# xuyuan/waymo_2d_tracking

Measured on AMD Instinct MI355X. Metric: end-to-end frames/sec (detect+SORT) on 1920x1280 Waymo frames, higher is better.
Workload: dtype f32; 1 GPU; Cascade R-CNN X152-32x8d-FPN dconv (random-init, fp32, batch 1) on synthetic 1920x1280x3 frames -> top-100 detections/frame -> SORT (max_age 2, min_hits 0, all boxes tracked; trackers resident for the whole segment); 5 cameras x 2 frames per step per GPU; 1x1 and dense 3x3 convolutions: f32 operands as exact 3 x bf16 splits, six cross terms on the bf16 matrix cores, f32 accumulate (csrc/det_gemm_s; stage=e2e, parallelism=sequence-shard x1

## Files before the change

### include/waymodet.h

```cpp
#ifndef WAYMODET_H
#define WAYMODET_H
#include <stddef.h>
#include <stdint.h>
#ifdef __cplusplus
extern "C" {
#endif

int wd_roi_pool_fpn_f32(const float* const* feats, const int32_t* heights, const int32_t* widths,
                        const float* scales, int n_levels, int channels, int batch,
                        const float* rois, int n_rois, int pooled, int min_level, int canonical_level,
                        float canonical_size, float* out, void* stream);

size_t wd_nms_workspace(int n);
int wd_select_kept(const uint8_t* keep_mask, const uint8_t* valid, const int64_t* order, int n, int cap, int64_t* out_idx,
                   int32_t* count, void* stream);
int wd_nms_sorted_f32(const float* boxes, const int32_t* idxs, int n, float iou_threshold,
                      uint8_t* keep_mask, int32_t* n_keep, void* workspace, size_t workspace_bytes, void* stream);

size_t wd_gemm_nt_workspace(int M, int N, int K);
int wd_gemm_nt_ws_f32(const float* A, const float* Bt, const float* bias, const float* residual, int relu, int M, int N, int K,
                      float* C, void* workspace, size_t workspace_bytes, void* stream);

int wd_gemm_lt_f32(const float* a, const float* w, const float* bias, const float* residual, float* out, int m, int n, int k,
                   int relu, void* workspace, size_t workspace_bytes, void* stream);
int wd_gemm_lt_plan_info(int m, int n, int k, int relu, int has_bias, int has_residual, float* best_us, int* candidates);
size_t wd_gemm_split_packed_bytes(int N, int K);
int wd_gemm_split_pack_weight(const float* w, int N, int K, void* packed, void* stream);
int wd_gemm_split_pack_weight_strided(const float* w, int N, int K, long stride_n, long stride_k, void* packed, void* stream);
typedef struct WdSplitPackDesc {
    const float* src;
    void* dst;
    long s_n, s_c, s_kh, s_kw;
    long first_block;
    int N, K, C, ksize, flip, reserved;
} WdSplitPackDesc;
int wd_gemm_split_pack_batch(const WdSplitPackDesc* descs_device, int count, long total_blocks, void* stream);
size_t wd_gemm_split_workspace(long M, int N, int K);
int wd_gemm_split_f32(const float* a, long lda, const void* packed_w, const float* bias, const float* residual, float* out, long ldc,
                      int M, int N, int K, int relu, void* workspace, size_t workspace_bytes, void* stream);
int wd_conv_split_f32(const float* x, int batch, int H, int W, int C, const void* packed_w, int ksize, int stride, int pad, const float* bias,
                      const float* residual, float* out, int N, int relu, void* workspace, size_t workspace_bytes, void* stream);
int wd_gemm_split_supported(const float* a, long lda, const float* bias, const float* residual, const float* out, long ldc, long M, int N, int K);
int wd_conv_split_position_major(int batch, int H, int W, int ksize, int stride, int pad);
typedef struct WdSplitIO {
    const float* a;
    long lda;
    const void* a_planes;
    const float* residual;
    const void* residual_planes;
    float* out;
    void* out_planes;
    long ldc;
} WdSplitIO;
size_t wd_split_planes_bytes(long M, int K);
int wd_split_planes_pack_f32(const float* a, long lda, long M, int K, void* planes, void* stream);
int wd_split_planes_unpack_f32(const void* planes, long M, int K, float* out, long ldo, void* stream);
int wd_gemm_split_io(const WdSplitIO* io, const void* packed_w, const float* bias, int M, int N, int K, int relu, void* workspace,
                     size_t workspace_bytes, void* stream);
int wd_nms_segmented_f32(const float* boxes, const int32_t* idxs, const int32_t* seg_offsets, int n_seg, float iou_threshold,
                         uint8_t* keep_mask, int32_t* n_keep, void* workspace, size_t workspace_bytes, void* stream);

size_t wd_rpn_topk_workspace(const int* n_per_level, int n_levels, int k);
int wd_rpn_topk_decode_f32(const float* const* logits, const float* const* deltas, const float* const* anchors,
                           const int* n_per_level, int n_levels, int k, float img_h, float img_w, float scale_clamp,
                           float* out_boxes, float* out_scores, int32_t* out_group, uint8_t* out_valid, void* workspace,
                           size_t workspace_bytes, void* stream);
int wd_sort_candidates_f32(const float* boxes, const float* scores, const int32_t* group, const uint8_t* valid,
                           const uint8_t* valid2 , int n, float* out_boxes, float* out_scores, int32_t* out_group, uint8_t* out_valid, int64_t* out_order,
                           void* stream);
int wd_box_candidates_f32(const float* boxes, const float* s0, const float* s1, const float* s2, const int32_t* n_valid, int rows,
                          int num_classes, float score_thresh, float img_h, float img_w, float* out_boxes, float* out_scores,
                          int32_t* out_group, uint8_t* out_valid, int64_t* out_order, void* stream);
int wd_gather_kept_f32(const uint8_t* keep, const uint8_t* valid, const float* boxes, const float* scores, const int64_t* order,
                       int n, int cap, int num_classes, float* out_boxes, float* out_scores, int64_t* out_class, int32_t* count,
                       void* stream);
int wd_detections_to_wire(const float* boxes, const float* scores, const int64_t* classes, const int32_t* count, int n, int in_w,
                          int in_h, int hflip, int out_w, int out_h, double* xywhs, int32_t* category, void* stream);

size_t wd_deform_packed_weight_floats(int c_in, int c_out, int groups);
int wd_deform_pack_weight(const float* weight_oihw, int c_in, int c_out, int groups, float* packed, void* stream);
const char* wd_deform_conv3x3_variant(int c_in, int groups, int stride, int pad, int has_offset);
int wd_deform_conv3x3_f32(const float* x, const float* offset, const float* mask, const float* packed_weight,
                          const float* scale, const float* bias, int relu,
                          int batch, int h, int w, int c_in, int c_out, int groups, int stride, int pad,
                          float* y, void* stream);
int wd_deform_conv3x3_hint_f32(const float* x, const float* offset, const float* mask, const float* packed_weight,
                               const float* scale, const float* bias, int relu, int batch, int h, int w, int c_in,
                               int c_out, int groups, int stride, int pad, int far_offsets, float* y, void* stream);
size_t wd_deform_table_bytes(int batch, int h, int w);
int wd_deform_offsets_table_f32(const float* partial, int ld, const float* bias, int batch, int h, int w, float* offsets,
                                void* table, void* stream);
int wd_deform_conv3x3_tab_f32(const float* x, const float* offset, const float* mask, const float* packed_weight,
                              const float* scale, const float* bias, int relu, int batch, int h, int w, int c_in,
                              int c_out, int groups, int stride, int pad, int far_offsets, const void* table, float* y,
                              void* stream);
// ... 57 lines not shown
```

### waymo_2d_tracking_amd/csrc/det_gemm_split.hip

```cpp
#include "common.h"
#include "../../include/waymodet.h"
#include <cstdlib>
#include <cstring>

namespace {

using bf16x8 = __attribute__((ext_vector_type(8))) __bf16;
using bf16x2 = __attribute__((ext_vector_type(2))) __bf16;
using f32x2 = __attribute__((ext_vector_type(2))) float;
using f32x16 = __attribute__((ext_vector_type(16))) float;
using u32x4 = __attribute__((ext_vector_type(4))) unsigned;

constexpr int BK = 64;
constexpr int BN = 256;
constexpr int NTHREADS = 512;
constexpr int CHUNK = 6144;

struct SplitArgs {
    const float* a;
    const unsigned char* ap;
    const uint4* w;
    const float* bias;
    const float* residual;
    const unsigned char* resp;
    float* out;
    unsigned char* outp;
    long lda, ldc;
    int M, N, K, relu;
    int tiles_m, tiles_n;
    int splitk;
    float* part;
    long long* stamps;
    int H, W, C, Ho, Wo, stride, pad, ksize;
};

__device__ __forceinline__ unsigned pk_bf16(float a, float b) {
    const f32x2 v = {a, b};
    return __builtin_bit_cast(unsigned, __builtin_convertvector(v, bf16x2));
}

__device__ __forceinline__ void split_pair(float x0, float x1, unsigned& h, unsigned& m, unsigned& l) {
    h = pk_bf16(x0, x1);
    const float r0 = x0 - __uint_as_float(h << 16), r1 = x1 - __uint_as_float(h & 0xffff0000u);
    m = pk_bf16(r0, r1);
    const float s0 = r0 - __uint_as_float(m << 16), s1 = r1 - __uint_as_float(m & 0xffff0000u);
    l = pk_bf16(s0, s1);
}

__device__ __forceinline__ float bf_lo(unsigned v) { return __uint_as_float(v << 16); }
__device__ __forceinline__ float bf_hi(unsigned v) { return __uint_as_float(v & 0xffff0000u); }

__device__ __forceinline__ size_t planes_offset(int row, int col, int ncols) {
    return ((size_t)(row >> 5) * (size_t)(ncols >> 5) + (size_t)(col >> 5)) * CHUNK +
           (size_t)((row & 31) * 64 + ((((col >> 3) & 3) ^ ((row >> 2) & 3)) << 4) + ((col >> 2) & 1) * 8);
}

// ... 490 lines not shown
    if ((j_) < ND) { dma_piece(kt + 3, (unsigned)wr, (j_)); }
    RD(rofs0, 2) RD(rofs0, 1) RD(rofs0, 0)
    SB;
    int cur = 0, nxt = BUF, nx2 = 2 * BUF, wr = 3 * BUF;
    for (int kt = 0; kt < nk; ++kt) {
        const int a1 = cur + rofs1, a0n = nxt + rofs0;
        WAITW(0, ND + 3);
        MF(2, 0, 0) RD(a1, 2) SB;
        MF(1, 1, 0) SB;
        MF(1, 0, 0) RD(a1, 1) SB;
        MF(0, 2, 0) SB;
        MF(0, 1, 0) SB;
        MF(0, 0, 0) RD(a1, 0) w_load(2 * kt + 2, 0); SB;
        WAITW(1, 3);
        MF(2, 0, 1) RD(a0n, 2) SB;
        MF(1, 1, 1) DMA(0) DMA(3) SB;
        MF(1, 0, 1) RD(a0n, 1) SB;
        MF(0, 2, 1) DMA(1) DMA(4) SB;
        MF(0, 1, 1) DMA(2) SB;
        MF(0, 0, 1) RD(a0n, 0) w_load(2 * kt + 3, 1); SB;
        __builtin_amdgcn_s_barrier();
        SB;
        const int t = cur; cur = nxt; nxt = nx2; nx2 = wr; wr = t;
    }
#undef DMA
#undef WAITW
#ifdef WD_DEBUG
    if (p.stamps) t_epi = __builtin_amdgcn_s_memtime();
#endif
    asm volatile("s_waitcnt vmcnt(0) lgkmcnt(0)" ::: "memory");
    __builtin_amdgcn_s_barrier();
    if (p.splitk > 1) {
        SplitArgs q = p;
        q.out = p.part + (size_t)kz * p.M * p.N;
        q.ldc = p.N;
        q.bias = nullptr; q.residual = nullptr; q.resp = nullptr; q.outp = nullptr; q.relu = 0;
        split_epilogue<MT>(q, smem, acc, m0, n0, wave, lane, p.M);
    } else {
        split_epilogue<MT>(p, smem, acc, m0, n0, wave, lane, p.M);
    }
#ifdef WD_DEBUG
    if (p.stamps && tid == 0) {
        long long* o = p.stamps + 8 * (long)blockIdx.x;
        o[0] = t_start; o[1] = t_main; o[2] = t_epi; o[3] = __builtin_amdgcn_s_memtime();
        o[4] = id_stamp; o[5] = __builtin_amdgcn_s_getreg(20  | (0 << 6) | (3 << 11));
        o[6] = r_start; o[7] = __builtin_amdgcn_s_memrealtime();
    }
#endif
}
#undef SB
#undef MF
#undef RD

__global__ __launch_bounds__(256) void split_planes_pack_kernel(const float* __restrict__ a, long lda, int M, int K, unsigned char* __restrict__ out, long total) {
    const long t = (long)blockIdx.x * 256 + threadIdx.x;
    if (t >= total) return;
    const int k8 = K / 8;
    const int row = (int)(t / k8), kq = (int)(t - (long)row * k8);
    float4 v0 = make_float4(0.f, 0.f, 0.f, 0.f), v1 = v0;
    if (row < M) {
        const float4* s = reinterpret_cast<const float4*>(a + (size_t)row * lda + 8 * kq);
        v0 = s[0]; v1 = s[1];
    }
    unsigned h[4], m[4], l[4];
    split_pair(v0.x, v0.y, h[0], m[0], l[0]); split_pair(v0.z, v0.w, h[1], m[1], l[1]);
    split_pair(v1.x, v1.y, h[2], m[2], l[2]); split_pair(v1.z, v1.w, h[3], m[3], l[3]);
    unsigned char* q = out + planes_offset(row, 8 * kq, K);
    *reinterpret_cast<uint4*>(q) = make_uint4(h[0], h[1], h[2], h[3]);
    *reinterpret_cast<uint4*>(q + 2048) = make_uint4(m[0], m[1], m[2], m[3]);
    *reinterpret_cast<uint4*>(q + 4096) = make_uint4(l[0], l[1], l[2], l[3]);
}

__global__ __launch_bounds__(256) void split_planes_unpack_kernel(const unsigned char* __restrict__ planes, int M, int K, float* __restrict__ out, long ldo, long total) {
    const long t = (long)blockIdx.x * 256 + threadIdx.x;
    if (t >= total) return;
    const int k8 = K / 8;
    const int row = (int)(t / k8), kq = (int)(t - (long)row * k8);
    const unsigned char* q = planes + planes_offset(row, 8 * kq, K);
    const uint4 h = *reinterpret_cast<const uint4*>(q), m = *reinterpret_cast<const uint4*>(q + 2048), l = *reinterpret_cast<const uint4*>(q + 4096);
    float4* d = reinterpret_cast<float4*>(out + (size_t)row * ldo + 8 * kq);
    d[0] = make_float4((bf_lo(h.x) + bf_lo(m.x)) + bf_lo(l.x), (bf_hi(h.x) + bf_hi(m.x)) + bf_hi(l.x), (bf_lo(h.y) + bf_lo(m.y)) + bf_lo(l.y),
                       (bf_hi(h.y) + bf_hi(m.y)) + bf_hi(l.y));
    d[1] = make_float4((bf_lo(h.z) + bf_lo(m.z)) + bf_lo(l.z), (bf_hi(h.z) + bf_hi(m.z)) + bf_hi(l.z), (bf_lo(h.w) + bf_lo(m.w)) + bf_lo(l.w),
                       (bf_hi(h.w) + bf_hi(m.w)) + bf_hi(l.w));
}

__global__ __launch_bounds__(256) void gemm_split_pack_kernel(const float* __restrict__ w, int N, int K, long sn, long sk, uint4* __restrict__ out, long total) {
    const long t = (long)blockIdx.x * 256 + threadIdx.x;
    if (t >= total) return;
    const int k8 = K / 8;
    const int n = (int)(t / k8), kq = (int)(t - (long)n * k8);
    float v[8];
#pragma unroll
    for (int e = 0; e < 8; ++e) v[e] = n < N ? w[(size_t)n * sn + (size_t)(8 * kq + e) * sk] : 0.f;
    unsigned h[4], m[4], l[4];
#pragma unroll
    for (int e = 0; e < 4; ++e) split_pair(v[2 * e], v[2 * e + 1], h[e], m[e], l[e]);
    const int nt = n >> 5, ks = kq >> 1, ln = (n & 31) + 32 * (kq & 1);
    uint4* dst = out + ((size_t)nt * (K / 16) + ks) * 192 + ln;
    dst[0] = make_uint4(h[0], h[1], h[2], h[3]);
    dst[64] = make_uint4(m[0], m[1], m[2], m[3]);
    dst[128] = make_uint4(l[0], l[1], l[2], l[3]);
}

__global__ __launch_bounds__(256) void gemm_split_pack_batch_kernel(const WdSplitPackDesc* __restrict__ descs, int count) {
    int lo = 0, hi = count - 1;
// ... 155 lines not shown
    if (pl.splitk > 1 && workspace_bytes < (size_t)pl.splitk * a.M * a.N * sizeof(float)) pl = pick_plan(a.M, a.N, a.K, false);
    const int mt = pl.mt;
    a.splitk = pl.splitk;
    a.part = pl.splitk > 1 ? (float*)workspace : nullptr;
    a.tiles_m = (a.M + 32 * mt - 1) / (32 * mt);
    a.tiles_n = (a.N + BN - 1) / BN;
    int rc;
    switch (mt) {
        case 2: rc = launch<2, MODE>(a, stream); break;
        case 3: rc = launch<3, MODE>(a, stream); break;
        case 4: rc = launch<4, MODE>(a, stream); break;
        case 6: rc = launch<6, MODE>(a, stream); break;
        default: rc = launch<5, MODE>(a, stream); break;
    }
    if (rc != WT_OK || a.splitk == 1) return rc;
    const long mn4 = (long)a.M * a.N / 4;
    hipLaunchKernelGGL(gemm_split_reduce_kernel, dim3((unsigned)((mn4 + 255) / 256)), dim3(256), 0, stream, (const float4*)a.part, a.splitk, mn4, a.N / 4,
                       (const float4*)a.bias, a.residual, a.resp, a.ldc, a.relu, a.out, a.outp);
    WT_HIP(hipGetLastError());
    return WT_OK;
}

int dispatch_position_major(SplitArgs& a, hipStream_t stream) {
#ifdef WD_DEBUG
    a.stamps = g_stamps;
#endif
    const int maps = a.M / (a.H * a.W), kc = a.C / 32;
    const long tn = (a.N + BN - 1) / BN;
    const long ni = (long)(a.H - 2) * (a.W - 2), ne = 2l * (a.W - 2) + 2l * (a.H - 2);
    int best = 4;
    double best_t = 1e30;
    static const int forced_mt = experiment_knob("WD_SPLIT_MT");
    for (int mt = MT_MAX; mt >= MT_MIN; --mt) {
        if (forced_mt >= MT_MIN && forced_mt <= MT_MAX && mt != forced_mt) continue;
        const long nch = (maps + 32 * mt - 1) / (32 * mt);
        const double eff = (mt == 4 || mt == 5) ? 1.0 : 1.24;
        auto tile = [&](int taps) { return mt * taps * kc * 0.52 * eff + 2.0 + mt; };
        const double work = (double)nch * tn * (ni * tile(9) + ne * tile(6) + 4 * tile(4)) / 256.0;
        const double t = work > tile(9) ? work : tile(9);
        if (t < best_t * 0.97) { best_t = t; best = mt; }
    }
    a.splitk = 1; a.part = nullptr;
    a.tiles_m = a.H * a.W * ((maps + 32 * best - 1) / (32 * best));
    a.tiles_n = (int)tn;
    switch (best) {
        case 4: return launch<4, 3>(a, stream);
        case 6: return launch<6, 3>(a, stream);
        default: return launch<5, 3>(a, stream);
    }
}

bool misaligned(const void* p) { return (reinterpret_cast<uintptr_t>(p) & 15) != 0; }

}

extern "C" {

#ifdef WD_DEBUG
int wd_gemm_split_debug_stamps(long long* buf) {
    g_stamps = buf;
    return WT_OK;
}
#endif

size_t wd_gemm_split_packed_bytes(int N, int K) {
    if (N <= 0 || K <= 0 || (K % BK)) return 0;
    return (size_t)((N + 31) / 32) * 32 * (size_t)K * 6;
}

int wd_gemm_split_pack_weight_strided(const float* w, int N, int K, long stride_n, long stride_k, void* packed, void* stream_) {
    WT_TRY(wt::ensure_device());
    if (!w || !packed || N <= 0 || K <= 0 || (K % BK)) {
        wt::set_error("wd_gemm_split_pack_weight: K must be a positive multiple of %d (N=%d K=%d)", BK, N, K);
        return WT_ERR_INVALID;
    }
    const long total = (long)((N + 31) / 32) * 32 * (K / 8);
    hipLaunchKernelGGL(gemm_split_pack_kernel, dim3((unsigned)((total + 255) / 256)), dim3(256), 0, (hipStream_t)stream_, w, N, K, stride_n, stride_k,
                       (uint4*)packed, total);
    WT_HIP(hipGetLastError());
    return WT_OK;
}

int wd_gemm_split_pack_weight(const float* w, int N, int K, void* packed, void* stream_) {
    return wd_gemm_split_pack_weight_strided(w, N, K, (long)K, 1, packed, stream_);
}

int wd_gemm_split_pack_batch(const WdSplitPackDesc* descs_device, int count, long total_blocks, void* stream_) {
    WT_TRY(wt::ensure_device());
    if (count <= 0 || total_blocks <= 0) return WT_OK;
    if (!descs_device || total_blocks >= (1l << 31)) {
        wt::set_error("wd_gemm_split_pack_batch: NULL descriptor array or too many workgroups (%ld)", total_blocks);
        return WT_ERR_INVALID;
    }
    hipLaunchKernelGGL(gemm_split_pack_batch_kernel, dim3((unsigned)total_blocks), dim3(256), 0, (hipStream_t)stream_, descs_device, count);
    WT_HIP(hipGetLastError());
    return WT_OK;
}

size_t wd_gemm_split_workspace(long M, int N, int K) {
    if (M <= 0 || N <= 0 || K <= 0 || (K % BK) || (N % 32)) return 0;
    const Plan pl = pick_plan(M, N, K, true);
    return pl.splitk > 1 ? (size_t)pl.splitk * M * N * sizeof(float) : 0;
}

int wd_gemm_split_supported(const float* a, long lda, const float* bias, const float* residual, const float* out, long ldc, long M, int N, int K) {
    return M > 0 && N > 0 && K > 0 && (K % BK) == 0 && (N % 32) == 0 && (lda & 3) == 0 && (ldc & 3) == 0 && lda >= K && ldc >= N && !misaligned(a) &&
           !misaligned(bias) && !misaligned(residual) && !misaligned(out) && M < (1l << 31) && M * lda < (1l << 31);
}

int wd_gemm_split_f32(const float* a, long lda, const void* packed_w, const float* bias, const float* residual, float* out, long ldc,
                      int M, int N, int K, int relu, void* workspace, size_t workspace_bytes, void* stream_) {
    WT_TRY(wt::ensure_device());
    if (M <= 0 || N <= 0) return WT_OK;
    if (!a || !packed_w || !out || misaligned(packed_w) || !wd_gemm_split_supported(a, lda, bias, residual, out, ldc, M, N, K)) {
        wt::set_error("wd_gemm_split_f32: needs K %% %d == 0, N %% 32 == 0, 16-byte aligned rows and M * lda < 2^31 (M=%d N=%d K=%d lda=%ld)", BK, M, N,
                      K, lda);
        return WT_ERR_INVALID;
    }
    SplitArgs s{};
    s.a = a; s.w = (const uint4*)packed_w; s.bias = bias; s.residual = residual; s.out = out;
    s.lda = lda; s.ldc = ldc; s.M = M; s.N = N; s.K = K; s.relu = relu;
    return dispatch<0>(s, workspace, workspace_bytes, (hipStream_t)stream_);
}

size_t wd_split_planes_bytes(long M, int K) {
    if (M <= 0 || K <= 0 || (K % 32)) return 0;
    return (size_t)((M + 31) / 32) * (size_t)(K / 32) * CHUNK;
}

int wd_split_planes_pack_f32(const float* a, long lda, long M, int K, void* planes, void* stream_) {
    WT_TRY(wt::ensure_device());
    if (!a || !planes || M <= 0 || M >= (1l << 31) || K <= 0 || (K % 32) || (lda & 3) || lda < K || misaligned(a) || misaligned(planes)) {
        wt::set_error("wd_split_planes_pack_f32: needs K %% 32 == 0 and 16-byte aligned rows (M=%ld K=%d lda=%ld)", M, K, lda);
        return WT_ERR_INVALID;
    }
    const long total = ((M + 31) / 32) * 32 * (K / 8);
    hipLaunchKernelGGL(split_planes_pack_kernel, dim3((unsigned)((total + 255) / 256)), dim3(256), 0, (hipStream_t)stream_, a, lda, (int)M, K,
                       (unsigned char*)planes, total);
    WT_HIP(hipGetLastError());
    return WT_OK;
}

int wd_split_planes_unpack_f32(const void* planes, long M, int K, float* out, long ldo, void* stream_) {
    WT_TRY(wt::ensure_device());
    if (!out || !planes || M <= 0 || M >= (1l << 31) || K <= 0 || (K % 32) || (ldo & 3) || ldo < K || misaligned(out) || misaligned(planes)) {
        wt::set_error("wd_split_planes_unpack_f32: needs K %% 32 == 0 and 16-byte aligned rows (M=%ld K=%d ldo=%ld)", M, K, ldo);
        return WT_ERR_INVALID;
    }
    const long total = M * (K / 8);
    hipLaunchKernelGGL(split_planes_unpack_kernel, dim3((unsigned)((total + 255) / 256)), dim3(256), 0, (hipStream_t)stream_, (const unsigned char*)planes,
                       (int)M, K, out, ldo, total);
    WT_HIP(hipGetLastError());
    return WT_OK;
}

int wd_gemm_split_io(const WdSplitIO* io, const void* packed_w, const float* bias, int M, int N, int K, int relu, void* workspace,
                     size_t workspace_bytes, void* stream_) {
    WT_TRY(wt::ensure_device());
    if (M <= 0 || N <= 0) return WT_OK;
    if (!io || !packed_w || misaligned(packed_w) || (!io->a && !io->a_planes) || (io->a && io->a_planes) || (!io->out && !io->out_planes) ||
        (io->residual && io->residual_planes) || K <= 0 || (K % BK) || (N % 32) || misaligned(io->a_planes) || misaligned(io->residual_planes) ||
        misaligned(io->out_planes) ||
        !wd_gemm_split_supported(io->a ? io->a : (const float*)packed_w, io->a ? io->lda : K, bias, io->residual, io->out, io->ldc ? io->ldc : N, M, N, K)) {
        wt::set_error("wd_gemm_split_io: exactly one of a / a_planes, at least one of out / out_planes, at most one residual form; K %% %d == 0, "
                      "N %% 32 == 0, 16-byte aligned pointers and rows (M=%d N=%d K=%d)", BK, M, N, K);
        return WT_ERR_INVALID;
    }
    SplitArgs s{};
    s.a = io->a; s.ap = (const unsigned char*)io->a_planes; s.w = (const uint4*)packed_w; s.bias = bias;
    s.residual = io->residual; s.resp = (const unsigned char*)io->residual_planes; s.out = io->out; s.outp = (unsigned char*)io->out_planes;
    s.lda = io->a ? io->lda : K; s.ldc = io->ldc ? io->ldc : N; s.M = M; s.N = N; s.K = K; s.relu = relu;
    return io->a ? dispatch<0>(s, workspace, workspace_bytes, (hipStream_t)stream_) : dispatch<2>(s, workspace, workspace_bytes, (hipStream_t)stream_);
}

int wd_conv_split_position_major(int batch, int H, int W, int ksize, int stride, int pad) {
// ... 25 lines not shown
```

### waymo_2d_tracking_amd/detnet/nn/cascade_rcnn.py

```python
import math
import os

import torch
from torch import nn
import torch.nn.functional as F

from . import ops

BLOCKS = (3, 8, 36, 3)
STAGE_CH = (256, 512, 1024, 2048)
GROUPS = 32
PIXEL_MEAN = (103.530, 116.280, 123.675)
PIXEL_STD = (57.375, 57.120, 58.395)
SCALE_CLAMP = math.log(1000.0 / 16)


FUSED_TRAINING_EPILOGUES = True


SPLIT_GEMM = os.environ.get('WD_SPLIT_GEMM', '1') != '0'


OFFSET_SPLIT_MIN_ROWS = 30000


SPLIT_PLANES = os.environ.get('WD_SPLIT_PLANES', '0') == '1'
SPLIT_PLANES_MIN_CH = int(os.environ.get('WD_SPLIT_PLANES_MIN_CH', '1024'))


class PlanesAct:

    def __init__(self, planes, n, h, w, c):
        self.planes, self.n, self.h, self.w, self.c = planes, n, h, w, c


DECISION_LOG = None


def _split_ok(cin, cout):
    return SPLIT_GEMM and cin % 64 == 0 and cout % 32 == 0


class _PackedSplit:

    def __init__(self):
        self.buf = None
        self.key = None

    def get(self, weight):
        key = (weight.device, weight._version, weight.data_ptr())
        if self.buf is None or self.key != key:
            self.buf = ops.split_pack_weight(weight)
            self.key = key
        return self.buf


def _msra(shape, gen, fan_out=True):
    w = torch.empty(shape)
    fan = shape[0] * shape[2] * shape[3] if fan_out else shape[1] * shape[2] * shape[3]
    return w.normal_(0, math.sqrt(2.0 / fan), generator=gen)


class Conv1x1(nn.Module):

    def __init__(self, cin, cout, gen, bn_scale=1.0, bias=False):
        super().__init__()
        w = _msra((cout, cin, 1, 1), gen).view(cout, cin)
        s = bn_scale / math.sqrt(1.0 + 1e-5) if not bias else 1.0
        self.weight = nn.Parameter(w * s, requires_grad=False)
        self.bias = nn.Parameter(torch.zeros(cout), requires_grad=False)
        self._split = _PackedSplit()

    def forward(self, x, relu=False, residual=None, stride=1):
        if not torch.is_grad_enabled() and x.is_cuda and _split_ok(self.weight.shape[1], self.weight.shape[0]):
            pw = self._split.get(self.weight)
            cout = self.weight.shape[0]
# ... 55 lines not shown
            return ops.conv_split(x, self._split.get(self.weight), self.weight.shape[0], self.weight.shape[2], self.stride, self.pad,
                                  self.bias, None, relu)
        if not torch.is_grad_enabled() and self.weight.shape[0] % 4 == 0:
            y = F.conv2d(x, self.weight, None, self.stride, self.pad, 1, self.groups)
            if y.is_contiguous(memory_format=torch.channels_last):
                n, c, h, w = y.shape
                ops.bias_relu_(y.permute(0, 2, 3, 1).reshape(n * h * w, c), self.bias, relu)
                return y
            y = y + self.bias.view(1, -1, 1, 1)
            return F.relu_(y) if relu else y
        if (torch.is_grad_enabled() and ops.SPLIT_TRAIN and x.is_cuda and self.groups == 1 and self.weight.shape[2] in (1, 3)
                and _split_ok(self.weight.shape[1], self.weight.shape[0])):
            return ops.ConvSplitFn.apply(x, self.weight, self.bias, self.stride, self.pad, relu)
        y = F.conv2d(x, self.weight, self.bias, self.stride, self.pad, 1, self.groups)
        return F.relu_(y) if relu else y


class Bottleneck(nn.Module):

    def __init__(self, cin, cout, stride, deform, gen, offset_std):
        super().__init__()
        width = cout
        self.stride, self.deform = stride, deform
        self.shortcut = Conv1x1(cin, cout, gen) if cin != cout else None
        self.conv1 = Conv1x1(cin, width, gen)
        if deform:
            self.conv2_offset = ConvBN(width, 18, 3, stride, 1, 1, gen, bias=True)
            self.conv2_offset.weight.data.normal_(0, offset_std, generator=gen)
            w = _msra((width, width // GROUPS, 3, 3), gen)
            self.conv2_weight = nn.Parameter(w, requires_grad=False)
            self.conv2_scale = nn.Parameter(torch.full((width,), 1.0 / math.sqrt(1.0 + 1e-5)), requires_grad=False)
            self.conv2_bias = nn.Parameter(torch.zeros(width), requires_grad=False)
            self._packed = None
        else:
            self.conv2_weight = nn.Parameter(_msra((width, width // GROUPS, 3, 3), gen), requires_grad=False)
            self.conv2_scale = nn.Parameter(torch.full((width,), 1.0 / math.sqrt(1.0 + 1e-5)), requires_grad=False)
            self.conv2_bias = nn.Parameter(torch.zeros(width), requires_grad=False)
            self._packed = None
        self.conv3 = Conv1x1(width, cout, gen, bn_scale=0.25)

    def packed_weight(self):
        v = self.conv2_weight._version
        if self._packed is None or self._packed.device != self.conv2_weight.device or getattr(self, '_packed_v', -1) != v:
            self._packed = ops.deform_pack_weight(self.conv2_weight, GROUPS)
            self._packed_v = v
        return self._packed

    def offset_conv(self, x, deform_table=False, stride=1):
        w = self.conv2_offset.weight
        if getattr(self, '_off_w2', None) is None or self._off_w2.device != w.device or self._off_v != w._version:
            self._off_w2 = ops.tap_gemm_weight(w)
            self._off_v = w._version
        split = None
        if x.shape[0] * x.shape[2] * x.shape[3] >= OFFSET_SPLIT_MIN_ROWS and x.is_cuda and _split_ok(w.shape[1], 32):
            if getattr(self, '_off_split', None) is None or self._off_split_key != (w.device, w._version):
                w32 = ops.tap_gemm_weight(w, align=32)
                self._off_split, self._off_split_key = (ops.split_pack_weight(w32), w32.shape[0]), (w.device, w._version)
            split = self._off_split
        return ops.conv3x3_few(x, self._off_w2, self.conv2_offset.bias, 18, stride, deform_table, split=split)

    def forward(self, x, emit_planes=False):
        if isinstance(x, PlanesAct) or emit_planes:
            return self._forward_planes(x, emit_planes)
        sc = x if self.shortcut is None else self.shortcut(x, stride=self.stride)
        out = self.conv1(x, relu=True)
        rec = DECISION_LOG
        if rec is not None:
            out1, offset = out, None
        if self.deform and torch.is_grad_enabled():
            offset = self.conv2_offset(out)
            if FUSED_TRAINING_EPILOGUES and not (self.conv2_scale.requires_grad or self.conv2_bias.requires_grad):
                out = ops.DeformConvFn.apply(out, offset, self.conv2_weight, GROUPS, self.stride, 1, self.conv2_scale, self.conv2_bias, True)
            else:
                out = ops.DeformConvFn.apply(out, offset, self.conv2_weight, GROUPS, self.stride, 1)
                out = F.relu(out * self.conv2_scale.view(1, -1, 1, 1) + self.conv2_bias.view(1, -1, 1, 1))
        elif self.deform:
            table = None
            if self.stride == 1 and self.conv2_weight.shape[1] in (16, 32):
                offset, table = self.offset_conv(out, deform_table=True)
            else:
                offset = self.offset_conv(out, stride=self.stride)
            out = ops.deform_conv3x3(out, offset, self.packed_weight(), GROUPS, self.stride, 1, self.conv2_scale,
                                     self.conv2_bias, relu=True, table=table)
        else:
            out = ops.deform_conv3x3(out, None, self.packed_weight(), GROUPS, self.stride, 1, self.conv2_scale,
                                     self.conv2_bias, relu=True)
        if rec is None:
            return self.conv3(out, relu=True, residual=sc)
        out3 = self.conv3(out, relu=True, residual=sc)
        rec.append((out1.detach().clone(), None if offset is None else offset.detach().clone(), out.detach().clone(), out3.detach().clone(), self.stride))
        return out3


def _bottleneck_forward_planes(self, x, emit_planes):
    in_planes = isinstance(x, PlanesAct)
    cout = self.conv3.weight.shape[0]
    if in_planes:
        assert self.shortcut is None and self.stride == 1
        n, h, w, cin = x.n, x.h, x.w, x.c
        m = n * h * w
        o1, _ = ops.gemm_split_io(m, self.conv1.weight.shape[0], cin, self.conv1._split.get(self.conv1.weight), a_planes=x.planes, bias=self.conv1.bias, relu=True)
        out = o1.view(n, h, w, -1).permute(0, 3, 1, 2)
        sc = None
    else:
        sc = x if self.shortcut is None else self.shortcut(x, stride=self.stride)
        out = self.conv1(x, relu=True)
    table = None
    if self.stride == 1 and self.conv2_weight.shape[1] in (16, 32):
        offset, table = self.offset_conv(out, deform_table=True)
    else:
# ... 317 lines not shown
```

### waymo_2d_tracking_amd/detnet/nn/ops.py

```python
import ctypes as C
import os

import torch

from ... import _lib


EVENT_LOG = None


_RAW_STREAM = getattr(torch._C, '_cuda_getCurrentRawStream', None)
_RAW_DEVICE = getattr(torch._C, '_cuda_getDevice', None)


def _stream():
    if _RAW_STREAM is not None and _RAW_DEVICE is not None:
        return C.c_void_p(_RAW_STREAM(_RAW_DEVICE()))
    return C.c_void_p(torch.cuda.current_stream().cuda_stream)


def _p(t):
    return C.c_void_p(t.data_ptr()) if t is not None else None


# ... 177 lines not shown
    n, c, h, w = x.shape
    out = torch.empty((n, c, 2 * h, 2 * w), dtype=torch.float32, device=x.device, memory_format=torch.channels_last)
    _lib.check(_lib.lib().wd_upsample2x_nhwc_f32(_p(x), C.c_int(n), C.c_int(h), C.c_int(w), C.c_int(c), _p(out), _stream()),
               'wd_upsample2x_nhwc_f32')
    return out


def groupnorm_relu_(x, weight, bias, groups, eps=1e-5, relu=True):
    assert x.is_contiguous(memory_format=torch.channels_last) and x.dtype == torch.float32
    r, c, h, w = x.shape
    _lib.check(_lib.lib().wd_groupnorm_relu_nhwc_f32(_p(x), _p(weight), _p(bias), C.c_int(r), C.c_int(h * w), C.c_int(c),
                                                     C.c_int(groups), C.c_float(eps), C.c_int(1 if relu else 0), _stream()),
               'wd_groupnorm_relu_nhwc_f32')
    return x


class GroupNormReluFn(torch.autograd.Function):

    @staticmethod
    def forward(ctx, x, weight, bias, groups, eps, relu):
        x = _nhwc(x)
        r, c, h, w = x.shape
        y = torch.empty_like(x, memory_format=torch.channels_last)
        _lib.check(_lib.lib().wd_groupnorm_relu_out_nhwc_f32(_p(x), _p(y), _p(weight), _p(bias), C.c_int(r), C.c_int(h * w), C.c_int(c),
                                                             C.c_int(groups), C.c_float(eps), C.c_int(1 if relu else 0), _stream()),
                   'wd_groupnorm_relu_out_nhwc_f32')
        ctx.save_for_backward(x, weight, bias)
        ctx.cfg = (groups, eps, bool(relu))
        return y

    @staticmethod
    def backward(ctx, dy):
        x, weight, bias = ctx.saved_tensors
        groups, eps, relu = ctx.cfg
        dy = _nhwc(dy)
        r, c, h, w = x.shape
        dx = torch.empty_like(x, memory_format=torch.channels_last)
        dg = torch.empty(c, dtype=torch.float32, device=x.device)
        db = torch.empty(c, dtype=torch.float32, device=x.device)
        _lib.check(_lib.lib().wd_groupnorm_relu_bwd_nhwc_f32(_p(x), _p(dy), _p(weight), _p(bias), C.c_int(r), C.c_int(h * w), C.c_int(c),
                                                             C.c_int(groups), C.c_float(eps), C.c_int(1 if relu else 0), _p(dx), _p(dg), _p(db),
                                                             _stream()), 'wd_groupnorm_relu_bwd_nhwc_f32')
        return dx, dg, db, None, None, None


def tap_gemm_weight(weight, align=16):
    n_out, c = weight.shape[0], weight.shape[1]
    ld = (9 * n_out + align - 1) // align * align
    w2 = torch.zeros((ld, c), dtype=torch.float32, device=weight.device)
    w2[:9 * n_out] = weight.detach().float().permute(2, 3, 0, 1).reshape(9 * n_out, c)
    return w2


def conv3x3_few(x, w2, bias, n_out, stride=1, deform_table=False, split=None):
    x = _nhwc(x)
    n, c, h, w = x.shape
    a = x.permute(0, 2, 3, 1).reshape(n * h * w, c)
    if split is not None:
        packed, ld = split
        partial = gemm_split(a, packed, ld)
        ld_partial = ld
    else:
        partial = torch.mm(a, w2.t())
        ld_partial = w2.shape[0]
    ho, wo = (h - 1) // stride + 1, (w - 1) // stride + 1
    out = torch.empty((n, n_out, ho, wo), dtype=torch.float32, device=x.device, memory_format=torch.channels_last)
    if deform_table:
        assert n_out == 18 and stride == 1
        lib = _lib.lib()
        table = torch.empty(int(lib.wd_deform_table_bytes(C.c_int(n), C.c_int(h), C.c_int(w))), dtype=torch.uint8, device=x.device)
        _lib.check(lib.wd_deform_offsets_table_f32(_p(partial), C.c_int(ld_partial), _p(bias), C.c_int(n), C.c_int(h), C.c_int(w),
                                                   _p(out), _p(table), _stream()), 'wd_deform_offsets_table_f32')
        return out, table
    _lib.check(_lib.lib().wd_tap_shift_add_f32(_p(partial), C.c_int(ld_partial), C.c_int(n_out), _p(bias), C.c_int(n), C.c_int(h),
                                               C.c_int(w), C.c_int(stride), _p(out), _stream()), 'wd_tap_shift_add_f32')
    return out


_LT_WS = {}


def gemm_lt(a, weight, bias=None, residual=None, relu=False, out=None):
    m, k = a.shape
    n = weight.shape[0]
    assert a.is_contiguous() and weight.is_contiguous() and weight.shape[1] == k
    if out is None:
        out = torch.empty((m, n), dtype=torch.float32, device=a.device)
    assert out.is_contiguous() and (residual is None or residual.is_contiguous())
    key = (a.device, torch.cuda.current_stream().cuda_stream)
    ws = _LT_WS.get(key)
    if ws is None:
        ws = _LT_WS[key] = torch.empty(64 << 20, dtype=torch.uint8, device=a.device)
    _lib.check(_lib.lib().wd_gemm_lt_f32(_p(a), _p(weight), _p(bias), _p(residual), _p(out), C.c_int(m), C.c_int(n), C.c_int(k),
                                         C.c_int(1 if relu else 0), _p(ws), C.c_size_t(ws.numel()), _stream()), 'wd_gemm_lt_f32')
    return out


def _split_log_begin():
    if EVENT_LOG is None:
        return None
    e0 = torch.cuda.Event(enable_timing=True)
    e0.record()
    return e0


def _split_log_end(e0, tag, m, n, k):
    if e0 is None:
        return
    e1 = torch.cuda.Event(enable_timing=True)
    e1.record()
    EVENT_LOG.append((tag, 12.0 * m * n * k, e0, e1))


_SPLIT_WS_BYTES = {}
# ... 661 lines not shown
```

Measured before the change: 43.72 frames/s.

## Add thin split-bf16 GEMM for deform offset taps with stride-2 parity classes

Adds a dedicated thin GEMM kernel for the 18-channel deformable-offset 3x3 tap GEMM (N<=192). It splits A into bf16 planes in shared memory and uses 32x32x16 bf16 MFMA with double buffering. For stride-2 convs, input pixels are grouped into four parity classes, and each class computes only the taps that contribute to strided outputs, skipping unneeded tap products. The row-count threshold for using the split path is removed, so small levels also use it. This adds extra launches per stride-2 conv and scattered output writes.

Result: no change. 43.42 frames/s (-0.7%).

```diff
diff --git a/include/waymodet.h b/include/waymodet.h
--- a/include/waymodet.h
+++ b/include/waymodet.h
@@ -41,6 +41,9 @@
 int wd_conv_split_f32(const float* x, int batch, int H, int W, int C, const void* packed_w, int ksize, int stride, int pad, const float* bias,
                       const float* residual, float* out, int N, int relu, void* workspace, size_t workspace_bytes, void* stream);
 int wd_gemm_split_supported(const float* a, long lda, const float* bias, const float* residual, const float* out, long ldc, long M, int N, int K);
+int wd_gemm_split_thin_f32(const float* a, long lda, const void* packed_w, float* partial, int ld, int M, int N, int K, void* stream);
+int wd_offset_taps_s2_split_f32(const float* x, int batch, int H, int W, int C, const void* const* packed_w, int n_out, float* partial, int ld,
+                                void* stream);
 int wd_conv_split_position_major(int batch, int H, int W, int ksize, int stride, int pad);
 typedef struct WdSplitIO {
     const float* a;
diff --git a/waymo_2d_tracking_amd/csrc/det_gemm_split.hip b/waymo_2d_tracking_amd/csrc/det_gemm_split.hip
--- a/waymo_2d_tracking_amd/csrc/det_gemm_split.hip
+++ b/waymo_2d_tracking_amd/csrc/det_gemm_split.hip
@@ -2,6 +2,7 @@
 #include "../../include/waymodet.h"
 #include <cstdlib>
 #include <cstring>
+#include <type_traits>
 
 namespace {
 
@@ -598,6 +599,148 @@
 #undef MF
 #undef RD
 
+struct ThinArgs {
+    const float* a;
+    const uint4* w;
+    float* out;
+    long lda;
+    int M, K, ld;
+    int ncb, ncols;
+    int H, W, hc, wc, py, px;
+    int group, ntaps;
+    unsigned taps;
+};
+
+__device__ __forceinline__ long thin_row(const ThinArgs& p, int m) {
+    if (p.H == 0) return m;
+    const int hw = p.hc * p.wc;
+    const int b = m / hw, r = m - b * hw;
+    const int yy = r / p.wc, xx = r - yy * p.wc;
+    return ((long)b * p.H + 2 * yy + p.py) * p.W + 2 * xx + p.px;
+}
+
+#define WD_THIN_VGPR_FLOOR "v167"
+
+template <int RB>
+__global__ __launch_bounds__(NTHREADS) void gemm_split_thin_kernel(const ThinArgs p) {
+    constexpr int BM = 32 * RB;
+    constexpr int PLANE = BM * 64;
+    constexpr int BUF = 3 * PLANE;
+    constexpr int NLD = RB / 2;
+    constexpr int CG = 8 / RB;
+    __shared__ __attribute__((aligned(16))) unsigned char smem[2 * BUF];
+    asm volatile("" ::: WD_THIN_VGPR_FLOOR);
+    const int tid = threadIdx.x, lane = tid & 63;
+    const int wave = __builtin_amdgcn_readfirstlane(tid >> 6);
+    const int m0 = blockIdx.x * BM;
+    const int rb = wave % RB, cg = wave / RB;
+    const int per = p.ncb / CG, rem = p.ncb % CG;
+    const int nj = per + (cg < rem ? 1 : 0);
+    const int cb0 = cg * per + (cg < rem ? cg : rem);
+    const int nk = p.K / 32;
+
+    const int sq = tid & 7;
+    const float* arow[NLD];
+    int soff[NLD];
+#pragma unroll
+    for (int i = 0; i < NLD; ++i) {
+        const int r = (tid >> 3) + 64 * i;
+        int m = m0 + r;
+        m = m < p.M ? m : p.M - 1;
+        arow[i] = p.a + thin_row(p, m) * p.lda + 4 * sq;
+        soff[i] = r * 64 + ((((sq >> 1) ^ ((r >> 2) & 3))) << 4) + (sq & 1) * 8;
+    }
+    auto a_fetch = [&](int kt, int i) -> float4 {
+        kt = kt < nk ? kt : nk - 1;
+        return *reinterpret_cast<const float4*>(arow[i] + (size_t)kt * 32);
+    };
+    auto a_store = [&](int bufoff, int i, const float4& v) {
+        unsigned h0, m0_, l0, h1, m1, l1;
+        split_pair(v.x, v.y, h0, m0_, l0);
+        split_pair(v.z, v.w, h1, m1, l1);
+        unsigned char* b = smem + bufoff + soff[i];
+        *reinterpret_cast<uint2*>(b) = make_uint2(h0, h1);
+        *reinterpret_cast<uint2*>(b + PLANE) = make_uint2(m0_, m1);
+        *reinterpret_cast<uint2*>(b + 2 * PLANE) = make_uint2(l0, l1);
+    };
+    float4 anext[NLD];
+#pragma unroll
+    for (int i = 0; i < NLD; ++i) a_store(0, i, a_fetch(0, i));
+#pragma unroll
+    for (int i = 0; i < NLD; ++i) anext[i] = a_fetch(1, i);
+
+    const int rr = lane & 31, rg = lane >> 5;
+    const int ro0 = (rb * 32 + rr) * 64 + ((((0 + rg) ^ ((rr >> 2) & 3))) << 4);
+    const int ro1 = (rb * 32 + rr) * 64 + ((((2 + rg) ^ ((rr >> 2) & 3))) << 4);
+
+    auto run = [&](auto njc) {
+        constexpr int NJ = decltype(njc)::value;
+        constexpr int NA = NJ > 0 ? NJ : 1;
+        f32x16 acc[NA];
+#pragma unroll
+        for (int j = 0; j < NA; ++j)
+#pragma unroll
+            for (int e = 0; e < 16; ++e) acc[j][e] = 0.f;
+        const uint4* wq[NA];
+#pragma unroll
+        for (int j = 0; j < NA; ++j) wq[j] = p.w + (size_t)(cb0 + j) * (size_t)(p.K / 16) * 192 + lane;
+        bf16x8 wf[2][NA][3];
+        auto w_load = [&](int sub, int slot) {
+            sub = sub < 2 * nk ? sub : 2 * nk - 1;
+#pragma unroll
+            for (int j = 0; j < NJ; ++j)
+#pragma unroll
+                for (int pl = 0; pl < 3; ++pl) wf[slot][j][pl] = __builtin_bit_cast(bf16x8, wq[j][(size_t)sub * 192 + pl * 64]);
+        };
+        auto sub_step = [&](int aoff, int slot) {
+            bf16x8 af[3];
+#pragma unroll
+            for (int pl = 0; pl < 3; ++pl) af[pl] = *reinterpret_cast<const bf16x8*>(smem + aoff + pl * PLANE);
+#define TERM(pa, pb)                                                                                          \
+    _Pragma("unroll") for (int j = 0; j < NJ; ++j)                                                          \
+        acc[j] = __builtin_amdgcn_mfma_f32_32x32x16_bf16(af[pa], wf[slot][j][pb], acc[j], 0, 0, 0);
+            TERM(2, 0) TERM(1, 1) TERM(1, 0) TERM(0, 2) TERM(0, 1) TERM(0, 0)
+#undef TERM
+        };
+        w_load(0, 0);
+        __syncthreads();
+        for (int kt = 0; kt < nk; ++kt) {
+            const int cur = (kt & 1) * BUF, nxt = BUF - cur;
+            if (kt + 1 < nk) {
+#pragma unroll
+                for (int i = 0; i < NLD; ++i) a_store(nxt, i, anext[i]);
+            }
+#pragma unroll
+            for (int i = 0; i < NLD; ++i) anext[i] = a_fetch(kt + 2, i);
+            if (NJ > 0) {
+                w_load(2 * kt + 1, 1);
+                sub_step(cur + ro0, 0);
+                w_load(2 * kt + 2, 0);
+                sub_step(cur + ro1, 1);
+            }
+            __syncthreads();
+        }
+#pragma unroll
+        for (int j = 0; j < NJ; ++j) {
+            const int col = (cb0 + j) * 32 + rr;
+            if (col >= p.ncols) continue;
+            int oc = col;
+            if (p.ntaps > 0) {
+                const int ti = col / p.group;
+                oc = (int)((p.taps >> (4 * ti)) & 15u) * p.group + (col - ti * p.group);
+            }
+#pragma unroll
+            for (int e = 0; e < 16; ++e) {
+                const int m = m0 + rb * 32 + (e & 3) + 8 * (e >> 2) + 4 * rg;
+                if (m < p.M) p.out[(size_t)thin_row(p, m) * p.ld + oc] = acc[j][e];
+            }
+        }
+    };
+    if (nj == 2) run(std::integral_constant<int, 2>{});
+    else if (nj == 1) run(std::integral_constant<int, 1>{});
+    else run(std::integral_constant<int, 0>{});
+}
+
 __global__ __launch_bounds__(256) void split_planes_pack_kernel(const float* __restrict__ a, long lda, int M, int K, unsigned char* __restrict__ out, long total) {
     const long t = (long)blockIdx.x * 256 + threadIdx.x;
     if (t >= total) return;
@@ -859,6 +1002,30 @@
 
 bool misaligned(const void* p) { return (reinterpret_cast<uintptr_t>(p) & 15) != 0; }
 
+template <int RB>
+int launch_thin(const ThinArgs& a, hipStream_t stream) {
+    const void* fn = reinterpret_cast<const void*>(gemm_split_thin_kernel<RB>);
+    static wt::OncePerDevice attr;
+    const int dev = wt::device_index();
+    if (attr.needed(dev)) {
+        WT_TRY(occupancy_guard(fn, RB));
+        attr.mark(dev);
+    }
+    hipLaunchKernelGGL((gemm_split_thin_kernel<RB>), dim3((unsigned)((a.M + 32 * RB - 1) / (32 * RB))), dim3(NTHREADS), 0, stream, a);
+    WT_HIP(hipGetLastError());
+    return WT_OK;
+}
+
+int dispatch_thin(ThinArgs& a, hipStream_t stream) {
+    a.ncb = (a.ncols + 31) / 32;
+    return a.ncb >= 4 ? launch_thin<2>(a, stream) : launch_thin<4>(a, stream);
+}
+
+bool thin_args_bad(const float* a, long lda, const void* packed_w, const float* partial, int ld, long M, int N, int K) {
+    return !a || !packed_w || !partial || misaligned(a) || misaligned(packed_w) || M <= 0 || M >= (1l << 31) || N <= 0 || N > 192 || ld < N || K <= 0 ||
+           (K % BK) || (lda & 3) || lda < K;
+}
+
 }
 
 extern "C" {
@@ -928,6 +1095,48 @@
     s.a = a; s.w = (const uint4*)packed_w; s.bias = bias; s.residual = residual; s.out = out;
     s.lda = lda; s.ldc = ldc; s.M = M; s.N = N; s.K = K; s.relu = relu;
     return dispatch<0>(s, workspace, workspace_bytes, (hipStream_t)stream_);
+}
+
+int wd_gemm_split_thin_f32(const float* a, long lda, const void* packed_w, float* partial, int ld, int M, int N, int K, void* stream_) {
+    WT_TRY(wt::ensure_device());
+    if (M <= 0 || N <= 0) return WT_OK;
+    if (thin_args_bad(a, lda, packed_w, partial, ld, M, N, K)) {
+        wt::set_error("wd_gemm_split_thin_f32: needs N <= 192, ld >= N, K%% %d == 0, lda %% 4 == 0 and 16-byte aligned a / packed_w (M=%d N=%d K=%d ld=%d)",
+                      BK, M, N, K, ld);
+        return WT_ERR_INVALID;
+    }
+    ThinArgs t{};
+    t.a = a; t.w = (const uint4*)packed_w; t.out = partial; t.lda = lda; t.M = M; t.K = K; t.ld = ld; t.ncols = N;
+    return dispatch_thin(t, (hipStream_t)stream_);
+}
+
+int wd_offset_taps_s2_split_f32(const float* x, int batch, int H, int W, int C, const void* const* packed_w, int n_out, float* partial, int ld,
+                                void* stream_) {
+    WT_TRY(wt::ensure_device());
+    if (batch <= 0 || H <= 0 || W <= 0) return WT_OK;
+    if (!packed_w || n_out <= 0 || 4 * n_out > 192 || ld < 9 * n_out || (long)batch * H * W >= (1l << 31)) {
+        wt::set_error("wd_offset_taps_s2_split_f32: needs 4 n_out <= 192 and ld >= 9 n_out (n_out=%d ld=%d)", n_out, ld);
+        return WT_ERR_INVALID;
+    }
+    for (int cls = 0; cls < 4; ++cls) {
+        const int py = cls >> 1, px = cls & 1;
+        const int hc = (H - py + 1) / 2, wc = (W - px + 1) / 2;
+        const long M = (long)batch * hc * wc;
+        if (M == 0) continue;
+        ThinArgs t{};
+        for (int kh = 0; kh < 3; ++kh)
+            for (int kw = 0; kw < 3; ++kw)
+                if ((kh == 1) == (py == 0) && (kw == 1) == (px == 0)) t.taps |= (unsigned)(kh * 3 + kw) << (4 * t.ntaps++);
+        const int N = t.ntaps * n_out;
+        if (thin_args_bad(x, C, packed_w[cls], partial, ld, M, N, C)) {
+            wt::set_error("wd_offset_taps_s2_split_f32: needs C %% %d == 0 and 16-byte aligned x / packed_w[%d] (C=%d)", BK, cls, C);
+            return WT_ERR_INVALID;
+        }
+        t.a = x; t.w = (const uint4*)packed_w[cls]; t.out = partial; t.lda = C; t.M = (int)M; t.K = C; t.ld = ld; t.ncols = N;
+        t.H = H; t.W = W; t.hc = hc; t.wc = wc; t.py = py; t.px = px; t.group = n_out;
+        WT_TRY(dispatch_thin(t, (hipStream_t)stream_));
+    }
+    return WT_OK;
 }
 
 size_t wd_split_planes_bytes(long M, int K) {
diff --git a/waymo_2d_tracking_amd/detnet/nn/cascade_rcnn.py b/waymo_2d_tracking_amd/detnet/nn/cascade_rcnn.py
--- a/waymo_2d_tracking_amd/detnet/nn/cascade_rcnn.py
+++ b/waymo_2d_tracking_amd/detnet/nn/cascade_rcnn.py
@@ -19,9 +19,6 @@
 
 
 SPLIT_GEMM = os.environ.get('WD_SPLIT_GEMM', '1') != '0'
-
-
-OFFSET_SPLIT_MIN_ROWS = 30000
 
 
 SPLIT_PLANES = os.environ.get('WD_SPLIT_PLANES', '0') == '1'
@@ -183,10 +180,10 @@
             self._off_w2 = ops.tap_gemm_weight(w)
             self._off_v = w._version
         split = None
-        if x.shape[0] * x.shape[2] * x.shape[3] >= OFFSET_SPLIT_MIN_ROWS and x.is_cuda and _split_ok(w.shape[1], 32):
+        if x.is_cuda and _split_ok(w.shape[1], 32):
             if getattr(self, '_off_split', None) is None or self._off_split_key != (w.device, w._version):
-                w32 = ops.tap_gemm_weight(w, align=32)
-                self._off_split, self._off_split_key = (ops.split_pack_weight(w32), w32.shape[0]), (w.device, w._version)
+                s2 = ops.offset_s2_pack_weights(w) if self.stride == 2 else None
+                self._off_split, self._off_split_key = (ops.split_pack_weight(self._off_w2), s2), (w.device, w._version)
             split = self._off_split
         return ops.conv3x3_few(x, self._off_w2, self.conv2_offset.bias, 18, stride, deform_table, split=split)
 
diff --git a/waymo_2d_tracking_amd/detnet/nn/ops.py b/waymo_2d_tracking_amd/detnet/nn/ops.py
--- a/waymo_2d_tracking_amd/detnet/nn/ops.py
+++ b/waymo_2d_tracking_amd/detnet/nn/ops.py
@@ -253,14 +253,53 @@
     return w2
 
 
+def gemm_split_thin(a, packed, n, ld=None):
+    m, k = a.shape
+    ld = n if ld is None else ld
+    assert a.dtype == torch.float32 and a.stride(1) == 1
+    partial = torch.empty((m, ld), dtype=torch.float32, device=a.device)
+    e0 = _split_log_begin()
+    _lib.check(_lib.lib().wd_gemm_split_thin_f32(_p(a), C.c_long(a.stride(0)), _p(packed), _p(partial), C.c_int(ld), C.c_int(m), C.c_int(n), C.c_int(k),
+                                                 _stream()), 'wd_gemm_split_thin_f32')
+    _split_log_end(e0, 'gemm_split_thin_kernel: offset taps %dx%dx%d' % (m, n, k), m, (n + 31) // 32 * 32, k)
+    return partial
+
+
+S2_CLASS_TAPS = tuple(tuple(kh * 3 + kw for kh in ((1,) if py == 0 else (0, 2)) for kw in ((1,) if px == 0 else (0, 2)))
+                      for py in (0, 1) for px in (0, 1))
+
+
+def offset_s2_pack_weights(weight):
+    w = weight.detach().float()
+    n_out, c = w.shape[0], w.shape[1]
+    wt = w.permute(2, 3, 0, 1).reshape(9, n_out, c)
+    return tuple(split_pack_weight(wt[list(taps)].reshape(len(taps) * n_out, c).contiguous()) for taps in S2_CLASS_TAPS)
+
+
+def offset_taps_s2(x, packs, n_out, ld):
+    n, c, h, w = x.shape
+    partial = torch.empty((n * h * w, ld), dtype=torch.float32, device=x.device)
+    if _DEBUG_FILL:
+        partial.fill_(float('nan'))
+    ptrs = (C.c_void_p * 4)(*[pk.data_ptr() for pk in packs])
+    e0 = _split_log_begin()
+    _lib.check(_lib.lib().wd_offset_taps_s2_split_f32(_p(x), C.c_int(n), C.c_int(h), C.c_int(w), C.c_int(c), ptrs, C.c_int(n_out), _p(partial),
+                                                      C.c_int(ld), _stream()), 'wd_offset_taps_s2_split_f32')
+    _split_log_end(e0, 'gemm_split_thin_kernel: offset taps s2 %dx%dx%d' % (n * h * w, 9 * n_out, c), n * h * w // 4, 8 * 32, c)
+    return partial
+
+
 def conv3x3_few(x, w2, bias, n_out, stride=1, deform_table=False, split=None):
     x = _nhwc(x)
     n, c, h, w = x.shape
     a = x.permute(0, 2, 3, 1).reshape(n * h * w, c)
     if split is not None:
-        packed, ld = split
-        partial = gemm_split(a, packed, ld)
-        ld_partial = ld
+        packed, s2_packs = split
+        ld_partial = w2.shape[0]
+        if stride == 2 and s2_packs is not None:
+            partial = offset_taps_s2(x, s2_packs, n_out, ld_partial)
+        else:
+            partial = gemm_split_thin(a, packed, 9 * n_out, ld_partial)
     else:
         partial = torch.mm(a, w2.t())
         ld_partial = w2.shape[0]
```
